# PKU-MARL/HARL

Hardware: AMD Instinct MI355X
Metric: transitions/sec through HAPPO update (MPE spread, 3 agents) (higher is better)
Workload: dtype f32; 1 GPU; MPE simple_spread_v2 3-agent HAPPO update: compute_returns + train(), T=200, n_rollout_threads=4096/GPU (4096 global, weak scaling), obs18/share54/Box5, MLP[128, 128], ppo_epoch=5, critic_epoch=5; episode_length=200, n_rollout_threads_per_gpu=4096, n_rollout_threads_global=4096, n_agents=3, parallelism=dp1, collective=none, world_size=1, ranks_seen=1

## Files before the change

harl_amd/csrc/common.h:

```cpp
#pragma once
#include <hip/hip_runtime.h>
#include <stdint.h>

typedef float f32x16 __attribute__((ext_vector_type(16)));
typedef float f32x4 __attribute__((ext_vector_type(4)));

#ifdef HARL_PHASE_TIMING
#define HARL_NPHASE 12
static __device__ long long harl_phase_cyc[8][HARL_NPHASE];
static __device__ long long harl_phase_wg[8][256][3];
#define PHASE_BEGIN()                                    \
  long long _pt_acc[HARL_NPHASE];                        \
  for (int _k = 0; _k < HARL_NPHASE; ++_k) _pt_acc[_k] = 0; \
  const long long _pt_rt0 = __builtin_amdgcn_s_memrealtime(); \
  const long long _pt_c0 = __builtin_readcyclecounter(); \
  long long _pt_last = _pt_c0;
#define PHASE(i)                                         \
  do {                                                   \
    __builtin_amdgcn_sched_barrier(0);                   \
    const long long _t = __builtin_readcyclecounter();   \
    _pt_acc[i] += _t - _pt_last;                         \
    _pt_last = _t;                                       \
    __builtin_amdgcn_sched_barrier(0);                   \
  } while (0)
#define PHASE_END(slot)                                  \
  do {                                                   \
    if (blockIdx.x == 0 && threadIdx.x == 0)             \
      for (int _k = 0; _k < HARL_NPHASE; ++_k) harl_phase_cyc[slot][_k] = _pt_acc[_k]; \
    if (threadIdx.x == 0 && blockIdx.x < 256) {          \
      harl_phase_wg[slot][blockIdx.x][0] = __builtin_readcyclecounter() - _pt_c0; \
      harl_phase_wg[slot][blockIdx.x][1] = _pt_rt0;      \
      harl_phase_wg[slot][blockIdx.x][2] = __builtin_amdgcn_s_memrealtime(); \
    }                                                    \
  } while (0)
#define HARL_PHASE_ACCESSOR(tu)                                                                    \
  extern "C" int harl_phase_read_##tu(long long *out) {                                            \
    return (int)hipMemcpyFromSymbol(out, HIP_SYMBOL(harl_phase_cyc), sizeof(long long) * 8 * HARL_NPHASE); \
  }                                                                                                \
  extern "C" int harl_phase_read_wg_##tu(long long *out) {                                         \
    return (int)hipMemcpyFromSymbol(out, HIP_SYMBOL(harl_phase_wg), sizeof(long long) * 8 * 256 * 3); \
  }
#else
#define PHASE_BEGIN()
#define PHASE(i)
#define PHASE_END(slot)
#define HARL_PHASE_ACCESSOR(tu)
#endif

namespace harl {

constexpr int WAVE = 64;
constexpr int SLAB = 32;
constexpr int WG_THREADS = 256;
constexpr int WAVES_PER_WG = 4;
constexpr int PS_STRIDE = 48;
constexpr int DHEAD_LD = 32;

void set_error(const char *msg);
int check_launch(const char *what);

__device__ __forceinline__ constexpr int feat_base(int R) {
  return 32 * (R >> 4) + (R & 3) + 8 * ((R & 15) >> 2);
}

#ifdef HARL_NO_WAVE_ID
__device__ __forceinline__ int wave_id() { return (int)(threadIdx.x >> 6); }
#else
__device__ __forceinline__ int wave_id() { return __builtin_amdgcn_readfirstlane((int)(threadIdx.x >> 6)); }
#endif
__device__ __forceinline__ float uniform_f(float v) {
  return __uint_as_float(__builtin_amdgcn_readfirstlane(__float_as_uint(v)));
}
__device__ __forceinline__ float wave_xor32(float v) {
  return __shfl_xor(v, 32, 64);
}
__device__ __forceinline__ float wave_sum32(float v) {
  const unsigned u = __float_as_uint(v);
  const auto r = __builtin_amdgcn_permlane32_swap(u, u, false, false);
  return __uint_as_float(r[0]) + __uint_as_float(r[1]);
}

__device__ __forceinline__ float half_reduce_sum(float v) {
#pragma unroll
  for (int o = 16; o >= 1; o >>= 1) v += __shfl_xor(v, o, 64);
  return v;
}
__device__ __forceinline__ float wave_reduce_sum(float v) {
#pragma unroll
  for (int o = 32; o >= 1; o >>= 1) v += __shfl_xor(v, o, 64);
  return v;
}
__device__ __forceinline__ double wave_reduce_sum_d(double v) {
#pragma unroll
  for (int o = 32; o >= 1; o >>= 1) v += __shfl_xor(v, o, 64);
  return v;
}

template <int H>
__device__ __forceinline__ void atl_load(const float *__restrict__ base, long slab, int lane, float (&x)[H / 2]) {
  const f32x4 *p = reinterpret_cast<const f32x4 *>(base + slab * (long)(H * SLAB)) + lane;
#pragma unroll
  for (int q = 0; q < H / 8; ++q) {
    f32x4 v = p[q * WAVE];
    x[4 * q + 0] = v[0];
    x[4 * q + 1] = v[1];
    x[4 * q + 2] = v[2];
    x[4 * q + 3] = v[3];
  }
}
template <int H>
__device__ __forceinline__ void atl_store(float *__restrict__ base, long slab, int lane, const float (&x)[H / 2]) {
  f32x4 *p = reinterpret_cast<f32x4 *>(base + slab * (long)(H * SLAB)) + lane;
#pragma unroll
  for (int q = 0; q < H / 8; ++q) {
    f32x4 v;
    v[0] = x[4 * q + 0];
    v[1] = x[4 * q + 1];
    v[2] = x[4 * q + 2];
    v[3] = x[4 * q + 3];
    p[q * WAVE] = v;
  }
}

#ifndef HARL_NO_PK
typedef float f32x2 __attribute__((ext_vector_type(2)));
__device__ __forceinline__ f32x2 fma2(f32x2 a, f32x2 b, f32x2 c) { return __builtin_elementwise_fma(a, b, c); }
#ifdef HARL_PK_SPLIT_OFF
constexpr bool PK_DEFAULT = false;
// ... 135 lines not shown
```

harl_amd/csrc/mfma_transpose.h:

```cpp
#pragma once
#include "split_mfma.h"

namespace harl {

constexpr unsigned BF16_ONE_LO = 0x00003F80u, BF16_ONE_HI = 0x3F800000u;

struct Ident {
  u32x4 j0, j1;
};
__device__ __forceinline__ Ident make_ident(int lane) {
  const int n = lane & 31, g = lane >> 5;
  Ident I;
#pragma unroll
  for (int c = 0; c < 4; ++c) {
    const int f0 = ((2 * c) & 3) + 8 * ((2 * c) >> 2) + 4 * g, f1 = f0 + 1;
    I.j0[c] = (n == f0 ? BF16_ONE_LO : 0u) | (n == f1 ? BF16_ONE_HI : 0u);
    I.j1[c] = (n == 16 + f0 ? BF16_ONE_LO : 0u) | (n == 16 + f1 ? BF16_ONE_HI : 0u);
  }
  return I;
}
__device__ __forceinline__ u32x4 make_ident16(int lane) {
  const int n = lane & 31, g = lane >> 5;
  u32x4 I;
#pragma unroll
  for (int c = 0; c < 4; ++c) I[c] = (n == 8 * g + 2 * c ? BF16_ONE_LO : 0u) | (n == 8 * g + 2 * c + 1 ? BF16_ONE_HI : 0u);
  return I;
}

__device__ __forceinline__ unsigned pack_hi16(float lo, float hi) {
  return __builtin_amdgcn_perm(__float_as_uint(hi), __float_as_uint(lo), 0x07060302u);
}

__device__ __forceinline__ void pack_transposed(const f32x16 &acc, u32x4 &o0, u32x4 &o1) {
#pragma unroll
  for (int c = 0; c < 4; ++c) {
    o0[c] = pack_hi16(acc[2 * c], acc[2 * c + 1]);
    o1[c] = pack_hi16(acc[8 + 2 * c], acc[8 + 2 * c + 1]);
  }
}

template <bool SUM>
__device__ __forceinline__ float transpose_block(const u32x4 &x1a, const u32x4 &x1b, const u32x4 &x2a, const u32x4 &x2b,
                                                 const u32x4 &x3a, const u32x4 &x3b, const Ident &I, u32x4 (&T)[3][2]) {
  const f32x16 zero = {0.f, 0.f, 0.f, 0.f, 0.f, 0.f, 0.f, 0.f, 0.f, 0.f, 0.f, 0.f, 0.f, 0.f, 0.f, 0.f};
  f32x16 c1 = mfma_bf16(x1a, I.j0, zero), c2 = mfma_bf16(x2a, I.j0, zero), c3 = mfma_bf16(x3a, I.j0, zero);
  c1 = mfma_bf16(x1b, I.j1, c1);
  c2 = mfma_bf16(x2b, I.j1, c2);
  c3 = mfma_bf16(x3b, I.j1, c3);
  pack_transposed(c1, T[0][0], T[0][1]);
  pack_transposed(c2, T[1][0], T[1][1]);
  pack_transposed(c3, T[2][0], T[2][1]);
  float s = 0.f;
  if constexpr (SUM) {
    f32x2 a = {0.f, 0.f};
#pragma unroll
    for (int r = 0; r < 8; ++r) {
      a += f32x2{c3[2 * r], c3[2 * r + 1]};
      a += f32x2{c2[2 * r], c2[2 * r + 1]};
      a += f32x2{c1[2 * r], c1[2 * r + 1]};
    }
    s = a[0] + a[1];
  }
  return s;
}

template <bool SUM, bool PACKED = PK_DEFAULT>
__device__ __forceinline__ float split_transpose_block(const float *v16, const Ident &I, u32x4 (&T)[3][2]) {
  u32x4 y1[2], y2[2], y3[2];
#pragma unroll
  for (int j = 0; j < 2; ++j)
#pragma unroll
    for (int c = 0; c < 4; ++c) {
      unsigned a, b, d;
      split3<PACKED>(v16[8 * j + 2 * c], v16[8 * j + 2 * c + 1], a, b, d);
      y1[j][c] = a;
      y2[j][c] = b;
      y3[j][c] = d;
    }
  return transpose_block<SUM>(y1[0], y1[1], y2[0], y2[1], y3[0], y3[1], I, T);
}

__device__ __forceinline__ void dw_tile(f32x16 &acc, const u32x4 (&A)[3][2], const u32x4 (&B)[3][2]) {
#pragma unroll
  for (int ks = 0; ks < 2; ++ks) {
    acc = mfma_bf16(A[2][ks], B[0][ks], acc);
    acc = mfma_bf16(A[0][ks], B[2][ks], acc);
    acc = mfma_bf16(A[1][ks], B[1][ks], acc);
    acc = mfma_bf16(A[1][ks], B[0][ks], acc);
    acc = mfma_bf16(A[0][ks], B[1][ks], acc);
    acc = mfma_bf16(A[0][ks], B[0][ks], acc);
  }
}

template <int MT_, int NT_>
__device__ __forceinline__ void finish_partials(f32x16 (&acc)[MT_][NT_], float (&db)[MT_], float *buf,
                                                float *__restrict__ part, int n_part_rows) {
  constexpr int HO = 32 * MT_, KP = 32 * NT_, ROW = HO * KP + HO;
  const int lane = threadIdx.x & 63, wave = wave_id(), i = lane & 31, h = lane >> 5;
  float dbt[MT_];
#pragma unroll
  for (int a = 0; a < MT_; ++a) dbt[a] = wave_sum32(db[a]);
  __syncthreads();
  for (int w = 0; w < WAVES_PER_WG; ++w) {
    if (wave == w) {
#pragma unroll
      for (int a = 0; a < MT_; ++a) {
#pragma unroll
        for (int b = 0; b < NT_; ++b)
#pragma unroll
          for (int r = 0; r < 16; ++r) {
            const int o = 32 * a + (r & 3) + 8 * (r >> 2) + 4 * h;
            float *p = buf + o * KP + 32 * b + i;
            *p = (w == 0 ? 0.f : *p) + acc[a][b][r];
          }
        if (h == 0) {
          float *p = buf + HO * KP + 32 * a + i;
          *p = (w == 0 ? 0.f : *p) + dbt[a];
        }
      }
    }
    __syncthreads();
  }
  float *out = part + (long)blockIdx.x * ROW;
  for (int e = threadIdx.x; e < ROW; e += WG_THREADS) out[e] = buf[e];
  for (int row = blockIdx.x + gridDim.x; row < n_part_rows; row += gridDim.x) {
    float *z = part + (long)row * ROW;
    for (int e = threadIdx.x; e < ROW; e += WG_THREADS) z[e] = 0.f;
  }
}

}
```

harl_amd/csrc/mlp.hip:

```cpp
#include "common.h"
#include "split_mfma.h"
#include "mfma_transpose.h"
#include "dw_common.h"
#include "fwd_epilogue.h"
#include "../../include/harl_hip.h"
#include <stdlib.h>
#include <type_traits>

using namespace harl;

#define MFMA(a, b, c) __builtin_amdgcn_mfma_f32_32x32x2f32((a), (b), (c), 0, 0, 0)

template <int HO>
__device__ __forceinline__ void ln_jac_store(f32x16 (&acc)[HO / 32], const float *__restrict__ xprimal,
                                             const uint32_t *__restrict__ mask_in, const float *__restrict__ rstd_in,
                                             int lane, long slab, float *__restrict__ xdot_out) {
  constexpr int NR = HO / 2, NW = (NR + 31) / 32;
  float xh[NR];
  atl_load<HO>(xprimal, slab, lane, xh);
  uint32_t bits[NW];
#pragma unroll
  for (int w = 0; w < NW; ++w) bits[w] = mask_in[(slab * NW + w) * WAVE + lane];
  const float rstd = rstd_in[slab * SLAB + (lane & 31)];
  float ad[NR];
// ... 1377 lines not shown
        constexpr int TSLOT = r == 0 ? 31 : 15;
        auto slot = [&](auto sc) {
          constexpr int s_ = decltype(sc)::value;
          if constexpr (r == 0) {
            if constexpr (s_ >= 16 && s_ < 32) a_chunk(s_ - 16);
            else if constexpr (s_ >= 32 && s_ < 42) b_chunk(s_ - 32 + 6);
            else if constexpr (s_ >= 42) p_chunk(s_ - 42);
            if constexpr (s_ == 41) d_load_next(ds2, base);
          } else {
            if constexpr (s_ < 16) a_chunk(s_);
            else if constexpr (s_ < 26) b_chunk(s_ - 16 + 6);
            else if constexpr (s_ < 32) p_chunk(s_ - 26);
            else if constexpr (!OSPLIT_IN_GEMM) {
              o_chunk(O_FIRST + s_ - 32, false);
              if constexpr (s_ - 32 < O_EXTRA) o_chunk(O_FIRST + 16 + s_ - 32, true);
            } else if constexpr (r == 3 && s_ < 40) {
              o_chunk(s_ - 32, false);
            }
            if constexpr (s_ == 25 && r < 3) d_load_next(ds2, base);
          }
          if constexpr (s_ == TSLOT) {
            static_for<0, 6>([&](auto kc) {
              constexpr int k = decltype(kc)::value;
              __builtin_amdgcn_sched_barrier(0);
              t_mfma(k);
              b_chunk(k);
            });
          }
        };
        u32x4 bv[2][3];
        read_frag(r & 1, 0, 0, bv[0]);
        if constexpr (!FILL) static_for<0, 48>(slot);
        static_for<0, 8>([&](auto nc) {
          constexpr int n = decltype(nc)::value, ks = n >> 2, b = n & 3;
          if constexpr (n + 1 < 8) read_frag(r & 1, (n + 1) >> 2, (n + 1) & 3, bv[(n + 1) & 1]);
          __builtin_amdgcn_sched_barrier(0);
          constexpr int AT[6] = {2, 0, 1, 1, 0, 0}, BT[6] = {0, 2, 1, 0, 1, 0};
          static_for<0, 6>([&](auto kc) {
            constexpr int k6 = decltype(kc)::value;
            acc2[b] = mfma_bf16(At[AT[k6]][ks], bv[n & 1][BT[k6]], acc2[b]);
            if constexpr (FILL) slot(std::integral_constant<int, 6 * n + k6>{});
            __builtin_amdgcn_sched_barrier(0);
          });
        });
        PHASE(6);
        b_store((r + 1) & 1);
#pragma unroll
        for (int t = 0; t < 3; ++t) {
          At[t][0] = AtN[t][0];
          At[t][1] = AtN[t][1];
        }
        PHASE(7);
      }
    });
  }

  {
    constexpr long ROW2 = (long)H * H + H;
    float *mypart = dw2_part + (long)blockIdx.x * ROW2;
#pragma unroll
    for (int b = 0; b < 4; ++b)
#pragma unroll
      for (int r = 0; r < 16; ++r) {
        const int o = 32 * wave + (r & 3) + 8 * (r >> 2) + 4 * h;
        mypart[(long)o * H + 32 * b + i] = acc2[b][r];
      }
    const float dbt = wave_sum32(db2);
    if (h == 0) mypart[(long)H * H + 32 * wave + i] = dbt;
    for (int row = blockIdx.x + gridDim.x; row < n_part_rows; row += gridDim.x) {
      float *z = dw2_part + (long)row * ROW2;
      for (int e = threadIdx.x; e < ROW2; e += WG_THREADS) z[e] = 0.f;
    }
  }
  if constexpr (KT > 0) {
    f32x16 a1x[4][1];
#pragma unroll
    for (int a = 0; a < 4; ++a) a1x[a][0] = acc1[a];
    finish_partials<4, 1>(a1x, dbs, reinterpret_cast<float *>(img), dw1_part, n_part_rows);
  }
  PHASE(11);
  PHASE_END(3);
}

HARL_PHASE_ACCESSOR(mlp)

static int bad(const char *m) {
  set_error(m);
  return -2;
}

extern "C" int harl_mlp_fwd_input(const float *X, long ldx, const int64_t *idx, long M, int D, const float *Wp,
                                  const float *bp, int use_ln0, int H, float *xout, uint32_t *relu_mask, float *rstd,
                                  float *mu0, float *rstd0, float *x0n, void *stream) {
  if (M <= 0) return 0;
  const long n_slabs = n_slabs_of(M);
  const int nch = (D + 31) / 32;
  const int grid = persistent_grid(n_slabs, 2);
  hipStream_t s = (hipStream_t)stream;
  if (H != 128 && H != 64) return bad("harl_mlp_fwd_input: hidden width must be 64 or 128");
  if (D <= 64) {
    const int kr = D <= 32 ? 32 : 64;
    const size_t shm = ((size_t)kr * H + H + (size_t)WAVES_PER_WG * SLAB * (kr + 1)) * sizeof(float);
#define LS(Hv, R)                                                                                                 \
  {                                                                                                               \
    allow_big_lds(k_fwd_input_staged<Hv, R>, shm);                                                                \
    hipLaunchKernelGGL((k_fwd_input_staged<Hv, R>), dim3(grid), dim3(WG_THREADS), shm, s, X, ldx, idx, M, D, Wp, bp, \
                       use_ln0, xout, relu_mask, rstd, mu0, rstd0, x0n, n_slabs);                                  \
  }
    if (H == 128) {
      if (D <= 32) LS(128, 2) else LS(128, 1)
    } else {
      if (D <= 32) LS(64, 2) else LS(64, 1)
    }
#undef LS
    return check_launch("harl_mlp_fwd_input");
  }
  const int resident = (long)nch * 32 * H * 4 <= 64 * 1024;
  const size_t shm = ((size_t)(resident ? nch * 32 : 32) * H + H) * sizeof(float);
  if (H == 128) {
    allow_big_lds(k_fwd_input<128, false>, shm);
    hipLaunchKernelGGL((k_fwd_input<128, false>), dim3(grid), dim3(WG_THREADS), shm, s, X, ldx, idx, M, D, Wp, bp,
                       use_ln0, xout, relu_mask, rstd, mu0, rstd0, n_slabs, nch, resident, nullptr, nullptr, nullptr);
  } else {
    allow_big_lds(k_fwd_input<64, false>, shm);
    hipLaunchKernelGGL((k_fwd_input<64, false>), dim3(grid), dim3(WG_THREADS), shm, s, X, ldx, idx, M, D, Wp, bp,
                       use_ln0, xout, relu_mask, rstd, mu0, rstd0, n_slabs, nch, resident, nullptr, nullptr, nullptr);
  }
  return check_launch("harl_mlp_fwd_input");
}

extern "C" int harl_mlp_tangent_input(const float *X, long ldx, const int64_t *idx, long M, int D, const float *Wdp,
                                      const float *bdp, int use_ln0, int H, const float *x1, const uint32_t *mask1,
                                      const float *rstd1, float *x1dot, void *stream) {
  if (M <= 0) return 0;
  const long n_slabs = n_slabs_of(M);
  const int nch = (D + 31) / 32;
  const int grid = persistent_grid(n_slabs, 2);
  hipStream_t s = (hipStream_t)stream;
  const int resident = (long)nch * 32 * H * 4 <= 64 * 1024;
  const size_t shm = ((size_t)(resident ? nch * 32 : 32) * H + H) * sizeof(float);
  if (H == 128) {
    allow_big_lds(k_fwd_input<128, true>, shm);
    hipLaunchKernelGGL((k_fwd_input<128, true>), dim3(grid), dim3(WG_THREADS), shm, s, X, ldx, idx, M, D, Wdp, bdp,
                       use_ln0, x1dot, nullptr, nullptr, nullptr, nullptr, n_slabs, nch, resident, x1, mask1, rstd1);
  } else if (H == 64) {
    allow_big_lds(k_fwd_input<64, true>, shm);
    hipLaunchKernelGGL((k_fwd_input<64, true>), dim3(grid), dim3(WG_THREADS), shm, s, X, ldx, idx, M, D, Wdp, bdp,
                       use_ln0, x1dot, nullptr, nullptr, nullptr, nullptr, n_slabs, nch, resident, x1, mask1, rstd1);
  } else {
    return bad("harl_mlp_tangent_input: hidden width must be 64 or 128");
  }
  return check_launch("harl_mlp_tangent_input");
}

extern "C" int harl_mlp_tangent_hidden(const float *xin_dot, const float *xin, long M, int HI, int HO, const float *Wp,
                                       const float *Wdp, const float *bdp, const float *xprimal,
                                       const uint32_t *mask_in, const float *rstd_in, float *xout_dot, void *stream) {
  if (M <= 0) return 0;
  const long n_slabs = n_slabs_of(M);
  const size_t shm = split_image_bytes(HO, HI) + (size_t)HO * sizeof(float);
  const int grid = persistent_grid(n_slabs, split_one_wg(HO, HI) ? 1 : 2);
  hipStream_t s = (hipStream_t)stream;
#define L(a, b)                                                                                                      \
  {                                                                                                                  \
    allow_big_lds(k_fwd_hidden<a, b, 1>, shm);                                                                       \
    hipLaunchKernelGGL((k_fwd_hidden<a, b, 1>), dim3(grid), dim3(WG_THREADS), shm, s, xin, Wdp, bdp, xout_dot, nullptr, \
// ... 131 lines not shown
  hipStream_t s = (hipStream_t)stream;
#define L(a, b)                                                                                                  \
  allow_big_lds(k_fwd_hidden<a, b>, shm);                                                                        \
  hipLaunchKernelGGL((k_fwd_hidden<a, b>), dim3(grid), dim3(WG_THREADS), shm, s, xin, Wp, bp, xout, relu_mask, rstd, \
                     n_slabs, nullptr, nullptr, nullptr)
  if (HI == 128 && HO == 128) { L(128, 128); }
  else if (HI == 64 && HO == 64) { L(64, 64); }
  else if (HI == 128 && HO == 64) { L(128, 64); }
  else if (HI == 64 && HO == 128) { L(64, 128); }
  else return bad("harl_mlp_fwd_hidden: widths must be 64 or 128");
#undef L
  return check_launch("harl_mlp_fwd_hidden");
}

static bool lean_bwd() {
  static const bool v = [] {
    const char *e = getenv("HARL_BWD_STREAMS");
    return e && e[0] == '1';
  }();
  return v;
}

extern "C" int harl_mlp_bwd_dx(const float *dz, const float *xprev, const uint32_t *relu_mask_prev,
                               const float *rstd_prev, long M, int HO, int HI, const float *Wp, float *dz_prev,
                               const float *x0n, int kp0, float *dw_part, int n_wg, void *stream) {
  if (M <= 0) return 0;
  const long n_slabs = n_slabs_of(M);
  hipStream_t s = (hipStream_t)stream;
  if (dw_part) {
    if (!x0n || (kp0 != 32 && kp0 != 64) || n_wg <= 0)
      return bad("harl_mlp_bwd_dx: fused first-layer gradient needs x0n, kp0 in {32, 64} and n_wg > 0");
#define LFX(a, b, kt, lean)                                                                                       \
  {                                                                                                               \
    size_t shm = split_image_bytes(b, a);                                                                         \
    const size_t rowb = ((size_t)b * 32 * kt + b) * sizeof(float);                                                \
    if (shm < rowb) shm = rowb;                                                                                   \
    allow_big_lds(k_bwd_dx<a, b, kt, lean>, shm);                                                                 \
    hipLaunchKernelGGL((k_bwd_dx<a, b, kt, lean>), dim3(n_wg < 256 ? n_wg : 256), dim3(WG_THREADS), shm, s, dz,   \
                       xprev, relu_mask_prev, rstd_prev, Wp, dz_prev, n_slabs, x0n, dw_part, n_wg);               \
  }
#define LF(a, b, kt) LFX(a, b, kt, false)
    const int kt = kp0 / 32;
    if (HO == 128 && HI == 128 && kt == 1 && lean_bwd()) LFX(128, 128, 1, true)
    else if (HO == 128 && HI == 128) { if (kt == 1) LF(128, 128, 1) else LF(128, 128, 2) }
    else if (HO == 64 && HI == 64) { if (kt == 1) LF(64, 64, 1) else LF(64, 64, 2) }
    else if (HO == 128 && HI == 64) { if (kt == 1) LF(128, 64, 1) else LF(128, 64, 2) }
    else if (HO == 64 && HI == 128) { if (kt == 1) LF(64, 128, 1) else LF(64, 128, 2) }
    else return bad("harl_mlp_bwd_dx: widths must be 64 or 128");
#undef LF
#undef LFX
    return check_launch("harl_mlp_bwd_dx");
  }
  const size_t shm = split_image_bytes(HI, HO);
  const int grid = persistent_grid(n_slabs, split_one_wg(HI, HO) ? 1 : 2);
#define L(a, b)                                                                                                    \
  allow_big_lds(k_bwd_dx<a, b>, shm);                                                                              \
  hipLaunchKernelGGL((k_bwd_dx<a, b>), dim3(grid), dim3(WG_THREADS), shm, s, dz, xprev, relu_mask_prev, rstd_prev, Wp, \
                     dz_prev, n_slabs, nullptr, nullptr, 0)
  if (HO == 128 && HI == 128) { L(128, 128); }
  else if (HO == 64 && HI == 64) { L(64, 64); }
  else if (HO == 128 && HI == 64) { L(128, 64); }
  else if (HO == 64 && HI == 128) { L(64, 128); }
  else return bad("harl_mlp_bwd_dx: widths must be 64 or 128");
#undef L
  return check_launch("harl_mlp_bwd_dx");
}

extern "C" int harl_mlp_bwd_dx_dw(const float *dz, const float *xprev, const uint32_t *relu_mask_prev,
                                  const float *rstd_prev, long M, int HO, int HI, const float *Wp, float *dz_prev,
                                  const float *x0n, int kp0, float *dw1_part, float *dw2_part, int n_wg, int fill,
                                  void *stream) {
  if (M <= 0) return 0;
  if (HO != 128 || HI != 128) return bad("harl_mlp_bwd_dx_dw: 128 x 128 layers only (the layer kernels take the other widths)");
  if (!dw2_part || n_wg <= 0) return bad("harl_mlp_bwd_dx_dw: needs the partial arena of dW' and n_wg > 0");
  const bool first = dw1_part != nullptr;
  if (first && (!x0n || kp0 != 32)) return bad("harl_mlp_bwd_dx_dw: the fused first-layer gradient needs x0n with kp0 = 32");
  if (!first && !dz_prev) return bad("harl_mlp_bwd_dx_dw: dz_prev is required when no first-layer gradient is fused");
  const long n_slabs = n_slabs_of(M);
  const long wgs = (n_slabs + WAVES_PER_WG - 1) / WAVES_PER_WG;
  int grid = n_wg < 256 ? n_wg : 256;
  if (wgs < grid) grid = (int)wgs;
  const size_t shm = bdw_lds_bytes();
  hipStream_t s = (hipStream_t)stream;
#define LB(kt, fl)                                                                                                    \
  {                                                                                                                   \
    allow_big_lds(k_bwd_dx_dw<kt, fl>, shm);                                                                          \
    hipLaunchKernelGGL((k_bwd_dx_dw<kt, fl>), dim3(grid), dim3(WG_THREADS), shm, s, dz, xprev, relu_mask_prev,       \
                       rstd_prev, Wp, dz_prev, n_slabs, x0n, dw1_part, dw2_part, n_wg);                              \
  }
  if (first) { if (fill) LB(1, true) else LB(1, false) }
  else { if (fill) LB(0, true) else LB(0, false) }
#undef LB
  return check_launch("harl_mlp_bwd_dx_dw");
}

template <int MT, int NT>
static void launch_dw_tr(const float *a, const float *b, long n_slabs, float *part, int K, int tile0, int n_wg, hipStream_t s) {
  const size_t shm = (size_t)3 * 8 * ((2 * MT * 128 + 8) + (2 * NT * 128 + 8));
  allow_big_lds(k_dw_tr<MT, NT>, shm);
  hipLaunchKernelGGL((k_dw_tr<MT, NT>), dim3(n_wg), dim3(WG_THREADS), shm, s, a, b, n_slabs, part, (long)K * SLAB, tile0, K);
}

template <int A_KIND, int B_KIND, int MT, int NT>
static void launch_dw(const float *a, const float *b, long ldx, const int64_t *idx, const float *mu0,
                      const float *rstd0, int K, long M, long n_slabs, float *part, int KP, int n_wg, int ny,
                      hipStream_t s) {
  const size_t shm = ((size_t)DW_S * ((32 * MT + 4) + (32 * NT + 4)) + 2 * DW_S) * sizeof(float);
  hipLaunchKernelGGL((k_dw<A_KIND, B_KIND, MT, NT>), dim3(n_wg, ny), dim3(WG_THREADS), shm, s, a, b, ldx, idx, mu0,
                     rstd0, K, M, n_slabs, part, KP);
}

extern "C" int harl_mlp_dw_partials(const float *a, int a_kind, int lda, int HO, const float *b, int b_kind, long ldx,
                                    const int64_t *idx, const float *mu0, const float *rstd0, int K, long M,
                                    float *part, int n_wg, void *stream) {
  if (M <= 0 || n_wg <= 0) return 0;
  const long n_slabs = n_slabs_of(M);
  const int KP = ((K + 31) / 32) * 32;
  hipStream_t s = (hipStream_t)stream;
  if (a_kind == 1 && lda != DHEAD_LD) return bad("harl_mlp_dw_partials: head gradient matrix must have row stride 32");
  const int MT = a_kind == 1 ? 1 : HO / 32;
  if (a_kind == 0 && HO != 64 && HO != 128 && HO != 256) return bad("harl_mlp_dw_partials: HO must be 64, 128 or 256");
  if (a_kind == 1 && HO > 32) return bad("harl_mlp_dw_partials: head width must be <= 32");
#define DW(AK, BK, MTv, NTv, ny) launch_dw<AK, BK, MTv, NTv>(a, b, ldx, idx, mu0, rstd0, K, M, n_slabs, part, KP, n_wg, ny, s)
  if (b_kind == 0) {
    const int NT = K / 32;
    if (K % 32 != 0 || K < 32) return bad("harl_mlp_dw_partials: ATL input width must be a multiple of 32");
#define DWS(MTv, NTv) launch_dw_tr<MTv, NTv>(a, b, n_slabs, part, K, tile0, n_wg, s);
    if (K > 128 || K == 96 || MT == 8) {
      if (K % 32 != 0 || K > 512 || (MT != 8 && MT != 4 && MT != 2)) return bad("harl_mlp_dw_partials: wide ATL input must be a multiple of 32, <= 512");
      const int ntiles = K / 32;
      const int gstep = MT == 8 ? 2 : (MT == 4 && ntiles > 4 ? (ntiles + (ntiles + 5) / 6 - 1) / ((ntiles + 5) / 6) : 4);
      for (int tile0 = 0; tile0 < ntiles; tile0 += gstep) {
        const int nt = ntiles - tile0 < gstep ? ntiles - tile0 : gstep;
        if (MT == 8) {
          if (nt == 2) DWS(8, 2) else DWS(8, 1)
        } else if (MT == 4) {
          if (nt == 6) DWS(4, 6) else if (nt == 5) DWS(4, 5) else
          if (nt == 4) DWS(4, 4) else if (nt == 3) DWS(4, 3) else if (nt == 2) DWS(4, 2) else DWS(4, 1)
        } else {
          if (nt == 4) DWS(2, 4) else if (nt == 3) DWS(2, 3) else if (nt == 2) DWS(2, 2) else DWS(2, 1)
        }
      }
      return check_launch("harl_mlp_dw_partials");
    }
    const int tile0 = 0;
    if (MT == 4 && NT == 1) DW(0, 0, 4, 1, 1);
    else if (MT == 2 && NT == 1) DW(0, 0, 2, 1, 1);
    else if (MT == 4 && NT == 4) DWS(4, 4)
    else if (MT == 4 && NT == 2) DWS(4, 2)
    else if (MT == 2 && NT == 4) DWS(2, 4)
    else if (MT == 2 && NT == 2) DWS(2, 2)
#undef DWS
    else if (MT == 1 && NT == 4) DW(1, 0, 1, 4, 1);
    else if (MT == 1 && NT == 2) DW(1, 0, 1, 2, 1);
    else return bad("harl_mlp_dw_partials: unsupported tile shape");
  } else {
    const int ktiles = KP / 32;
    if (a_kind != 0) return bad("harl_mlp_dw_partials: raw-input B operand needs an ATL A operand");
    if (ktiles == 1) {
      if (MT == 4) DW(0, 1, 4, 1, 1); else DW(0, 1, 2, 1, 1);
    } else if (ktiles == 2) {
      if (MT == 4) DW(0, 1, 4, 2, 1); else DW(0, 1, 2, 2, 1);
    } else {
      const int ny = (ktiles + 3) / 4;
      if (MT == 4) DW(0, 1, 4, 4, ny); else DW(0, 1, 2, 4, ny);
    }
  }
#undef DW
  return check_launch("harl_mlp_dw_partials");
}

extern "C" int harl_mlp_dw_partials_multi(int n, const float *const *a, const float *const *b, float *const *part, int HO,
// ... 67 lines not shown
```

Baseline: 49.85 million transitions/s.

## Split backward dx/dW kernel into dx-owner and dW-producer wave groups

```diff
diff --git a/harl_amd/csrc/common.h b/harl_amd/csrc/common.h
--- a/harl_amd/csrc/common.h
+++ b/harl_amd/csrc/common.h
@@ -23,11 +23,12 @@
     _pt_last = _t;                                       \
     __builtin_amdgcn_sched_barrier(0);                   \
   } while (0)
-#define PHASE_END(slot)                                  \
+#define PHASE_END(slot) PHASE_END_BY(slot, 0)
+#define PHASE_END_BY(slot, tid)                          \
   do {                                                   \
-    if (blockIdx.x == 0 && threadIdx.x == 0)             \
+    if (blockIdx.x == 0 && threadIdx.x == (tid))         \
       for (int _k = 0; _k < HARL_NPHASE; ++_k) harl_phase_cyc[slot][_k] = _pt_acc[_k]; \
-    if (threadIdx.x == 0 && blockIdx.x < 256) {          \
+    if (threadIdx.x == (tid) && blockIdx.x < 256) {      \
       harl_phase_wg[slot][blockIdx.x][0] = __builtin_readcyclecounter() - _pt_c0; \
       harl_phase_wg[slot][blockIdx.x][1] = _pt_rt0;      \
       harl_phase_wg[slot][blockIdx.x][2] = __builtin_amdgcn_s_memrealtime(); \
@@ -44,6 +45,7 @@
 #define PHASE_BEGIN()
 #define PHASE(i)
 #define PHASE_END(slot)
+#define PHASE_END_BY(slot, tid)
 #define HARL_PHASE_ACCESSOR(tu)
 #endif
 
diff --git a/harl_amd/csrc/mfma_transpose.h b/harl_amd/csrc/mfma_transpose.h
--- a/harl_amd/csrc/mfma_transpose.h
+++ b/harl_amd/csrc/mfma_transpose.h
@@ -92,7 +92,7 @@
   }
 }
 
-template <int MT_, int NT_>
+template <int MT_, int NT_, int NTHR = WG_THREADS>
 __device__ __forceinline__ void finish_partials(f32x16 (&acc)[MT_][NT_], float (&db)[MT_], float *buf,
                                                 float *__restrict__ part, int n_part_rows) {
   constexpr int HO = 32 * MT_, KP = 32 * NT_, ROW = HO * KP + HO;
@@ -122,10 +122,10 @@
     __syncthreads();
   }
   float *out = part + (long)blockIdx.x * ROW;
-  for (int e = threadIdx.x; e < ROW; e += WG_THREADS) out[e] = buf[e];
+  for (int e = threadIdx.x; e < ROW; e += NTHR) out[e] = buf[e];
   for (int row = blockIdx.x + gridDim.x; row < n_part_rows; row += gridDim.x) {
     float *z = part + (long)row * ROW;
-    for (int e = threadIdx.x; e < ROW; e += WG_THREADS) z[e] = 0.f;
+    for (int e = threadIdx.x; e < ROW; e += NTHR) z[e] = 0.f;
   }
 }
 
diff --git a/harl_amd/csrc/mlp.hip b/harl_amd/csrc/mlp.hip
--- a/harl_amd/csrc/mlp.hip
+++ b/harl_amd/csrc/mlp.hip
@@ -1483,6 +1483,356 @@
   PHASE_END(3);
 }
 
+#ifndef HARL_BWD_SPLIT_WAVES
+#define HARL_BWD_SPLIT_WAVES 1
+#endif
+template <int KT, bool FILL>
+__global__ __launch_bounds__(2 * WG_THREADS, 1) void k_bwd_dx_dw8(
+    const float *__restrict__ dz, const float *__restrict__ xprev, const uint32_t *__restrict__ mask_prev,
+    const float *__restrict__ rstd_prev, const float *__restrict__ Wp, float *__restrict__ dz_prev, long n_slabs,
+    const float *__restrict__ x0n, float *__restrict__ dw1_part, float *__restrict__ dw2_part, int n_part_rows) {
+  constexpr int H = 128, MT = 4, NJ = 8, NR = 64, KPF = 32, NTH = 2 * WG_THREADS;
+  extern __shared__ __attribute__((aligned(16))) float lds[];
+  PHASE_BEGIN();
+  u32x4 *img = reinterpret_cast<u32x4 *>(lds);
+  unsigned char *Bb = reinterpret_cast<unsigned char *>(img + 3 * MT * NJ * 64);
+  stage_split_matrix<H, H, true, NTH>(img, Wp);
+  __syncthreads();
+  const int lane = threadIdx.x & 63, wave_ = wave_id();
+  const int wave = wave_ & 3;
+  const bool owner = wave_ < WAVES_PER_WG;
+  const int i = lane & 31, h = lane >> 5;
+  const u32x4 *wl = img + lane;
+  const long sr_stride = (long)gridDim.x * WAVES_PER_WG;
+  const long base0 = (long)blockIdx.x * WAVES_PER_WG;
+  const Ident ident = make_ident(lane);
+
+  f32x16 acc2[4];
+  f32x16 acc1[KT > 0 ? 4 : 1];
+  float dbs[KT > 0 ? 4 : 1];
+  float db2 = 0.f;
+  auto zero_acc2 = [&]() {
+#pragma unroll
+    for (int b = 0; b < 4; ++b)
+#pragma unroll
+      for (int r = 0; r < 16; ++r) acc2[b][r] = 0.f;
+  };
+  auto zero_acc1 = [&]() {
+#pragma unroll
+    for (int a = 0; a < (KT > 0 ? 4 : 1); ++a) {
+      dbs[a] = 0.f;
+#pragma unroll
+      for (int r = 0; r < 16; ++r) acc1[a][r] = 0.f;
+    }
+  };
+
+  f32x4 prA[4], prB[4];
+  u32x2_t spB[4][3];
+  u32x4 ya[3][2];
+  f32x16 tc[3];
+  u32x4 At[3][2], AtN[3][2];
+  float rr0 = 0.f, rr1 = 0.f;
+  auto d_load = [&](long ds) {
+#pragma unroll
+    for (int u = 0; u < 4; ++u) {
+      prA[u] = (reinterpret_cast<const f32x4 *>(dz + ds * (long)(H * SLAB)) + lane)[(4 * wave + u) * WAVE];
+      prB[u] = (reinterpret_cast<const f32x4 *>(xprev + ds * (long)(H * SLAB)) + lane)[(4 * wave + u) * WAVE];
+    }
+  };
+  float vnext = 1.f;
+  auto d_load_next = [&](long ds, long fallback) { d_load(ds < n_slabs ? ds : fallback); };
+  auto a_chunk = [&](int k) {
+    const int pi = k >> 1, j = pi >> 2, c = pi & 3, u = pi >> 1, e = 2 * (pi & 1);
+    if ((k & 1) == 0) {
+      unsigned p1;
+      split_stage1(prA[u][e], prA[u][e + 1], p1, rr0, rr1);
+      ya[0][j][c] = p1;
+    } else {
+      unsigned p2, p3;
+      split_stage2(rr0, rr1, p2, p3);
+      ya[1][j][c] = p2;
+      ya[2][j][c] = p3;
+    }
+  };
+  auto b_chunk = [&](int k) {
+    const int u = k >> 2, c2 = (k >> 1) & 1;
+    if ((k & 1) == 0) {
+      unsigned p1;
+      split_stage1(prB[u][2 * c2], prB[u][2 * c2 + 1], p1, rr0, rr1);
+      spB[u][0][c2] = p1;
+    } else {
+      unsigned p2, p3;
+      split_stage2(rr0, rr1, p2, p3);
+      spB[u][1][c2] = p2;
+      spB[u][2][c2] = p3;
+    }
+  };
+  auto t_mfma = [&](int k) {
+    const f32x16 zero = {0.f, 0.f, 0.f, 0.f, 0.f, 0.f, 0.f, 0.f, 0.f, 0.f, 0.f, 0.f, 0.f, 0.f, 0.f, 0.f};
+    const int t = k % 3;
+    if (k < 3) tc[t] = mfma_bf16(ya[t][0], ident.j0, zero);
+    else tc[t] = mfma_bf16(ya[t][1], ident.j1, tc[t]);
+  };
+  auto p_chunk = [&](int k) {
+    if (k < 3) {
+      pack_transposed(tc[k], AtN[k][0], AtN[k][1]);
+    } else {
+      f32x2 a = {0.f, 0.f};
+#pragma unroll
+      for (int r = 0; r < 8; ++r) a += f32x2{tc[k - 3][2 * r], tc[k - 3][2 * r + 1]};
+      db2 += vnext * (a[0] + a[1]);
+    }
+  };
+  auto b_store = [&](int buf) {
+#pragma unroll
+    for (int u = 0; u < 4; ++u) {
+      const int q = 4 * wave + u;
+      unsigned char *d = Bb + buf * BDW_BUF + (i >> 2) * BDW_SQ + (2 * (q >> 2) + ((q & 3) >> 1)) * 128 + (i & 3) * 32 +
+                         (8 * (q & 1) + 4 * h) * 2;
+#pragma unroll
+      for (int term = 0; term < 3; ++term) *reinterpret_cast<u32x2_t *>(d + term * BDW_IMG) = spB[u][term];
+    }
+  };
+  const int p16 = lane & 15, g1b = (lane >> 4) & 1;
+  const int frag_lane = g1b * 128 + (p16 >> 2) * 32 + (p16 & 3) * 8;
+  auto read_frag = [&](int buf, int ks, int tile, u32x4 (&f)[3]) {
+#pragma unroll
+    for (int term = 0; term < 3; ++term) {
+      const unsigned char *fp = Bb + buf * BDW_BUF + term * BDW_IMG + (4 * ks + h) * BDW_SQ + 2 * tile * 128 + frag_lane;
+      const u32x2_t lo = tr_read(fp), hi = tr_read(fp + 2 * BDW_SQ);
+      f[term] = u32x4{lo[0], lo[1], hi[0], hi[1]};
+    }
+  };
+
+  float raw[NR];
+  u32x4 g1[NJ], g2[NJ], g3[NJ];
+  auto o_chunk = [&](int k) {
+    const int pi = k >> 1, j = pi >> 2, c = pi & 3;
+    if ((k & 1) == 0) {
+      unsigned p1;
+      split_stage1(raw[2 * pi], raw[2 * pi + 1], p1, rr0, rr1);
+      g1[j][c] = p1;
+    } else {
+      unsigned p2, p3;
+      split_stage2(rr0, rr1, p2, p3);
+      g2[j][c] = p2;
+      g3[j][c] = p3;
+    }
+  };
+  if (!owner && base0 < n_slabs) {
+    d_load(base0);
+#pragma unroll
+    for (int k = 0; k < 16; ++k) a_chunk(k);
+#pragma unroll
+    for (int k = 0; k < 6; ++k) t_mfma(k);
+#pragma unroll
+    for (int k = 0; k < 16; ++k) b_chunk(k);
+#pragma unroll
+    for (int k = 0; k < 6; ++k) p_chunk(k);
+#pragma unroll
+    for (int t = 0; t < 3; ++t) {
+      At[t][0] = AtN[t][0];
+      At[t][1] = AtN[t][1];
+    }
+    b_store(0);
+  }
+  PHASE(10);
+
+  auto o_part = [&](long base) {
+    const long slab = base + wave;
+    const bool own = slab < n_slabs;
+    constexpr int OB1 = KT > 0 ? 4 : 3, OB2 = KT > 0 ? NJ : 6, OB3 = KT > 0 ? NJ + 1 : NJ;
+    auto obar = [&](int k) {
+      if (base + k < n_slabs) __builtin_amdgcn_s_barrier();
+    };
+    if (own) {
+      constexpr int RAW_LEAD = 3;
+      auto raw_ks = [&](int j) {
+        const f32x4 *p = reinterpret_cast<const f32x4 *>(dz + slab * (long)(H * SLAB)) + lane;
+#pragma unroll
+        for (int c = 0; c < 2; ++c) {
+          const f32x4 v = p[(2 * j + c) * WAVE];
+#pragma unroll
+          for (int e = 0; e < 4; ++e) raw[8 * j + 4 * c + e] = v[e];
+        }
+      };
+#pragma unroll
+      for (int j = 0; j < RAW_LEAD; ++j) raw_ks(j);
+      obar(0);
+#pragma unroll
+      for (int k = 0; k < 8; ++k) o_chunk(k);
+      float xh[NR];
+      float rstd;
+      uint32_t mbits[2];
+      f32x4 x0r[KT > 0 ? KPF / 8 : 1];
+      auto x0_operands = [&]() {
+        if constexpr (KT > 0) {
+          const f32x4 *bp = reinterpret_cast<const f32x4 *>(x0n + slab * (long)(KPF * SLAB)) + lane;
+#pragma unroll
+          for (int q = 0; q < KPF / 8; ++q) x0r[q] = bp[q * WAVE];
+        }
+      };
+      auto ln_operands = [&]() {
+        atl_load<H>(xprev, slab, lane, xh);
+        rstd = rstd_prev[slab * SLAB + i];
+#pragma unroll
+        for (int w = 0; w < 2; ++w) mbits[w] = mask_prev[(slab * 2 + w) * WAVE + lane];
+      };
+      constexpr int LN_STEP = NJ;
+      f32x16 acc[MT];
+#pragma unroll
+      for (int t = 0; t < MT; ++t)
+#pragma unroll
+        for (int r = 0; r < 16; ++r) acc[t][r] = 0.f;
+      PHASE(0);
+      split_gemm_fill<MT, NJ>(wl, g1, g2, g3, acc, [&](int s_, int k6) {
+        const int j1 = s_ / MT + 1, q = (s_ % MT) * 6 + k6;
+        if (j1 < NJ && q % 3 == 0) o_chunk(8 * j1 + q / 3);
+        if (s_ % MT == 0 && k6 == 0 && j1 - 1 + RAW_LEAD < NJ) raw_ks(j1 - 1 + RAW_LEAD);
+        if (s_ % MT == MT - 1 && k6 == 5) {
+          if (j1 == LN_STEP) ln_operands();
+          if (j1 == OB1) obar(1);
+          if (j1 == OB2) obar(2);
+          if (j1 == OB3) obar(3);
+        }
+      });
+      PHASE(1);
+      float dx[NR];
+#pragma unroll
+      for (int R = 0; R < NR; ++R) dx[R] = acc[R >> 4][R & 15];
+      float out[NR];
+      ln_bwd_relu_mbits<H>(dx, xh, mbits, rstd, out);
+      if (dz_prev) atl_store<H>(dz_prev, slab, lane, out);
+      x0_operands();
+      if constexpr (OB3 == NJ + 1) obar(3);
+      PHASE(2);
+      if constexpr (KT > 0) {
+        float xr0[KPF / 2];
+#pragma unroll
+        for (int q = 0; q < KPF / 8; ++q) {
+          xr0[4 * q + 0] = x0r[q][0];
+          xr0[4 * q + 1] = x0r[q][1];
+          xr0[4 * q + 2] = x0r[q][2];
+          xr0[4 * q + 3] = x0r[q][3];
+        }
+        u32x4 a1[KPF / 16], a2[KPF / 16], a3[KPF / 16];
+        split_acts<KPF / 2>(xr0, a1, a2, a3);
+        u32x4 Bt[3][2];
+        transpose_block<false>(a1[0], a1[1], a2[0], a2[1], a3[0], a3[1], ident, Bt);
+#pragma unroll
+        for (int a = 0; a < 4; ++a) {
+          u32x4 A1[3][2];
+          dbs[a] += split_transpose_block<true>(&out[16 * a], ident, A1);
+          dw_tile(acc1[a], A1, Bt);
+        }
+        PHASE(3);
+      }
+    }
+    else {
+#pragma unroll
+      for (int k = 0; k < 4; ++k) obar(k);
+    }
+  };
+  auto d_part = [&](long base) {
+    d_load_next(base + 1, base);
+    PHASE(4);
+    static_for<0, 4>([&](auto rc) {
+      constexpr int r = decltype(rc)::value;
+      if (base + r < n_slabs) {
+        __syncthreads();
+        PHASE(5);
+        const long ds1 = r < 3 ? base + r + 1 : base + sr_stride;
+        const long ds2 = r < 2 ? base + r + 2 : base + sr_stride;
+        vnext = uniform_f(ds1 < n_slabs ? 1.f : 0.f);
+        constexpr int TSLOT = r == 0 ? 31 : 15;
+        auto slot = [&](auto sc) {
+          constexpr int s_ = decltype(sc)::value;
+          if constexpr (r == 0) {
+            if constexpr (s_ >= 16 && s_ < 32) a_chunk(s_ - 16);
+            else if constexpr (s_ >= 32 && s_ < 42) b_chunk(s_ - 32 + 6);
+            else if constexpr (s_ >= 42) p_chunk(s_ - 42);
+            if constexpr (s_ == 47) d_load_next(ds2, base);
+          } else {
+            if constexpr (s_ < 16) a_chunk(s_);
+            else if constexpr (s_ < 26) b_chunk(s_ - 16 + 6);
+            else if constexpr (s_ < 32) p_chunk(s_ - 26);
+            if constexpr (s_ == 31 && r < 3) d_load_next(ds2, base);
+          }
+          if constexpr (s_ == TSLOT) {
+            static_for<0, 6>([&](auto kc) {
+              constexpr int k = decltype(kc)::value;
+              __builtin_amdgcn_sched_barrier(0);
+              t_mfma(k);
+              b_chunk(k);
+            });
+          }
+        };
+        u32x4 bv[2][3];
+        read_frag(r & 1, 0, 0, bv[0]);
+        if constexpr (!FILL) static_for<0, 48>(slot);
+        static_for<0, 8>([&](auto nc) {
+          constexpr int n = decltype(nc)::value, ks = n >> 2, b = n & 3;
+          if constexpr (n + 1 < 8) read_frag(r & 1, (n + 1) >> 2, (n + 1) & 3, bv[(n + 1) & 1]);
+          __builtin_amdgcn_sched_barrier(0);
+          constexpr int AT[6] = {2, 0, 1, 1, 0, 0}, BT[6] = {0, 2, 1, 0, 1, 0};
+          static_for<0, 6>([&](auto kc) {
+            constexpr int k6 = decltype(kc)::value;
+            acc2[b] = mfma_bf16(At[AT[k6]][ks], bv[n & 1][BT[k6]], acc2[b]);
+            if constexpr (FILL) slot(std::integral_constant<int, 6 * n + k6>{});
+            __builtin_amdgcn_sched_barrier(0);
+          });
+        });
+        PHASE(6);
+        b_store((r + 1) & 1);
+#pragma unroll
+        for (int t = 0; t < 3; ++t) {
+          At[t][0] = AtN[t][0];
+          At[t][1] = AtN[t][1];
+        }
+        PHASE(7);
+      }
+    });
+  };
+  if (owner) {
+    zero_acc1();
+    for (long base = base0; base < n_slabs; base += sr_stride) o_part(base);
+    zero_acc2();
+  } else {
+    zero_acc2();
+    for (long base = base0; base < n_slabs; base += sr_stride) d_part(base);
+    zero_acc1();
+  }
+
+  {
+    constexpr long ROW2 = (long)H * H + H;
+    float *mypart = dw2_part + (long)blockIdx.x * ROW2;
+    if (!owner) {
+#pragma unroll
+      for (int b = 0; b < 4; ++b)
+#pragma unroll
+        for (int r = 0; r < 16; ++r) {
+          const int o = 32 * wave + (r & 3) + 8 * (r >> 2) + 4 * h;
+          mypart[(long)o * H + 32 * b + i] = acc2[b][r];
+        }
+      const float dbt = wave_sum32(db2);
+      if (h == 0) mypart[(long)H * H + 32 * wave + i] = dbt;
+    }
+    for (int row = blockIdx.x + gridDim.x; row < n_part_rows; row += gridDim.x) {
+      float *z = dw2_part + (long)row * ROW2;
+      for (int e = threadIdx.x; e < ROW2; e += NTH) z[e] = 0.f;
+    }
+  }
+  if constexpr (KT > 0) {
+    f32x16 a1x[4][1];
+#pragma unroll
+    for (int a = 0; a < 4; ++a) a1x[a][0] = acc1[a];
+    finish_partials<4, 1, NTH>(a1x, dbs, reinterpret_cast<float *>(img), dw1_part, n_part_rows);
+  }
+  PHASE(11);
+  PHASE_END_BY(4, 0);
+  PHASE_END_BY(5, 64 * WAVES_PER_WG);
+}
+
 HARL_PHASE_ACCESSOR(mlp)
 
 static int bad(const char *m) {
@@ -1780,12 +2130,21 @@
   if (wgs < grid) grid = (int)wgs;
   const size_t shm = bdw_lds_bytes();
   hipStream_t s = (hipStream_t)stream;
+#if HARL_BWD_SPLIT_WAVES
+#define LB(kt, fl)                                                                                                    \
+  {                                                                                                                   \
+    allow_big_lds(k_bwd_dx_dw8<kt, fl>, shm);                                                                         \
+    hipLaunchKernelGGL((k_bwd_dx_dw8<kt, fl>), dim3(grid), dim3(2 * WG_THREADS), shm, s, dz, xprev, relu_mask_prev,  \
+                       rstd_prev, Wp, dz_prev, n_slabs, x0n, dw1_part, dw2_part, n_wg);                              \
+  }
+#else
 #define LB(kt, fl)                                                                                                    \
   {                                                                                                                   \
     allow_big_lds(k_bwd_dx_dw<kt, fl>, shm);                                                                          \
     hipLaunchKernelGGL((k_bwd_dx_dw<kt, fl>), dim3(grid), dim3(WG_THREADS), shm, s, dz, xprev, relu_mask_prev,       \
                        rstd_prev, Wp, dz_prev, n_slabs, x0n, dw1_part, dw2_part, n_wg);                              \
   }
+#endif
   if (first) { if (fill) LB(1, true) else LB(1, false) }
   else { if (fill) LB(0, true) else LB(0, false) }
 #undef LB
```

Result: faster. 52.44 million transitions/s, median of 6 (+5.2%).
